# qitianwu/SGFormer

Hardware: NVIDIA H100
Metric: nodes/sec fwd+bwd (higher is better)
Workload: dtype bf16

## Files before the change

include/sgformer_b200.h:

```cpp
#ifndef SGFORMER_B200_H
#define SGFORMER_B200_H

#include <stddef.h>
#include <stdint.h>

#ifdef __cplusplus
extern "C" {
#endif

#define SGF_F32 0
#define SGF_BF16 1

#define SGF_ERR_ARG (-1)
#define SGF_ERR_UNSUPPORTED (-2)
#define SGF_ERR_DRIVER (-3)

const char* sgf_version(void);
int64_t sgf_launch_count(void);
int sgf_set_device(int device);

int sgf_csr_build_ws_bytes(int64_t nnz, int64_t n, size_t* bytes );
int sgf_csr_build(const int64_t* edge_index , int64_t nnz, int64_t n, int by_source,
                  int self_loop_mode, int64_t* rowptr , int32_t* col, float* dinv ,
                  void* ws, size_t ws_bytes, void* stream);
// ... 19 lines not shown
int sgf_add_self_loops(const int64_t* edge_index, int64_t nnz, int64_t n, int64_t* out_edge_index ,
                       void* stream);
int sgf_edge_symmetry(const int64_t* edge_index, int64_t nnz, int64_t n, uint64_t* out2, void* stream);
int sgf_csr_build_weighted_ws_bytes(int64_t nnz, int64_t n, size_t* bytes );
int sgf_csr_build_weighted(const int64_t* edge_index, const float* weight , int64_t nnz, int64_t n, int by_source,
                           int self_loop_mode, int64_t* rowptr, int32_t* col, int64_t* eid, float* val, float* dinv ,
                           void* ws, size_t ws_bytes, void* stream);
int sgf_edge_symmetry_weighted(const int64_t* edge_index, const float* weight, int64_t nnz, int64_t n, uint64_t* out2, void* stream);
int sgf_edge_weight_grad(const int64_t* rowptr, const int32_t* col, const int64_t* eid, int64_t n_rows, int h, int dtype,
                         const void* a, int64_t lda, const void* b, int64_t ldb, const void* y, int64_t ldy, const void* u, int64_t ldu,
                         const float* dinv, const int64_t* edge_index, int64_t nnz, float* loop_grad, float* out, void* stream);
int sgf_csr_subset_ws_bytes(int64_t n_sub, int64_t max_out_nnz, size_t* bytes);
int sgf_csr_subset(const int64_t* rowptr, const int32_t* col, int64_t n, const int64_t* subset, int64_t n_sub,
                   int32_t* node_map, int64_t* out_rowptr , int32_t* out_col, int64_t out_col_capacity,
                   float* dinv , int64_t* out_needed, void* ws, size_t ws_bytes, void* stream);

int sgf_spmm(const int64_t* rowptr, const int32_t* col, const float* row_scale, const void* x, int64_t ldx,
             void* y, int64_t ldy, int64_t n_rows, int h, int dtype,
             int64_t max_row_len ,
             void* stream);
int sgf_spmm_heavy(const int32_t* col, const float* row_scale, const void* x, int64_t ldx, void* y, int64_t ldy, int h,
                   int dtype, const int64_t* seg_start, const int32_t* seg_len, int64_t n_seg, float* partial,
                   const int64_t* heavy_rows, const int64_t* heavy_seg_ptr, int64_t n_heavy, void* stream);
int sgf_spmm_weighted(const int64_t* rowptr, const int32_t* col, const float* val, const float* row_scale, const void* x, int64_t ldx,
                      void* y, int64_t ldy, int64_t n_rows, int h, int dtype, int64_t max_row_len, void* stream);
int sgf_spmm_heavy_weighted(const int32_t* col, const float* val, const float* row_scale, const void* x, int64_t ldx, void* y,
                            int64_t ldy, int h, int dtype, const int64_t* seg_start, const int32_t* seg_len, int64_t n_seg,
                            float* partial, const int64_t* heavy_rows, const int64_t* heavy_seg_ptr, int64_t n_heavy, void* stream);
int sgf_spmm_sum(const int64_t* rowptr, const int32_t* col, const void* x, int64_t ldx, void* y, int64_t ldy, int64_t n_rows, int h,
                 int dtype, int64_t max_row_len, void* stream);
int sgf_spmm_heavy_sum(const int32_t* col, const void* x, int64_t ldx, void* y, int64_t ldy, int h, int dtype,
                       const int64_t* seg_start, const int32_t* seg_len, int64_t n_seg, float* partial, const int64_t* heavy_rows,
                       const int64_t* heavy_seg_ptr, int64_t n_heavy, void* stream);

#define SGF_GAT_MAX_HEADS 8
int sgf_gat_logits(const void* xp, int64_t ldx, int64_t n, int heads, int c, int dtype, const float* att_src, const float* att_dst,
                   float* a_src, float* a_dst, void* stream);
int sgf_gat_fwd(const int64_t* rowptr, const int32_t* col, const void* xp, int64_t ldx, const float* a_src, const float* a_dst,
                int64_t n, int heads, int c, int dtype, int mean, const float* bias, void* out, int64_t ldo, float* lse, float p,
                uint64_t seed, void* stream);
int sgf_gat_bwd(const int64_t* rowptr, const int32_t* col, const int64_t* rowptr_t, const int32_t* col_t, const void* xp, int64_t ldx,
                const float* a_src, const float* a_dst, const float* lse, const void* g, int64_t ldg, const float* att_src,
                const float* att_dst, int64_t n, int heads, int c, int dtype, int mean, float p, uint64_t seed, float* r_ws,
                float* da_src, float* da_dst, void* dxp, int64_t ldd, void* stream);
int sgf_dense_dropout(const float* x, int64_t ldx, int64_t rows, int64_t cols, float p, uint64_t seed, float* y, int64_t ldy,
                      void* stream);

int sgf_spmm_flagged(const int64_t* rowptr, const int32_t* col, const float* row_scale, const void* x, int64_t ldx, void* y,
                     int64_t ldy, int64_t n_rows, int h, int dtype, int64_t max_row_len, const uint32_t* flags, int64_t slot_rows,
                     int n_slots, void* stream);
int sgf_spmm_range(const int64_t* rowptr, const int32_t* col, const float* row_scale, const void* x, int64_t ldx, void* y,
                   int64_t ldy, int64_t n_rows, int h, int dtype, const int32_t* lo, const int32_t* hi, const float* part_in,
                   float* part_out, int64_t ld_part, void* stream);
int sgf_csr_row_splits(const int64_t* rowptr, const int32_t* col, int64_t n_rows, const int32_t* thresholds, int n_thr,
                       int32_t* splits, void* stream);
int sgf_signal(uint32_t* flag, uint32_t value, void* stream);
int sgf_memcpy_async(void* dst, const void* src, size_t bytes, void* stream);
int sgf_wait_flags(const uint32_t* flags, int n, void* stream);

#define SGF_MAX_SRC 4
#define SGF_MAX_SEG 16

#define SGF_EPI_AFFINE 0
#define SGF_EPI_ATTN_APPLY 1
#define SGF_EPI_ATTN_GRAM 2

// ... 176 lines not shown
```

sgformer_b200/_lib.py:

```python
import ctypes as C
import os

from . import _build

_i32, _i64, _f32, _u64, _vp, _sz = C.c_int32, C.c_int64, C.c_float, C.c_uint64, C.c_void_p, C.c_size_t
SGF_MAX_SRC, SGF_MAX_SEG = 4, 16
F32, BF16 = 0, 1
EPI_AFFINE, EPI_ATTN_APPLY, EPI_ATTN_GRAM = 0, 1, 2


class GemmNtArgs(C.Structure):
    _fields_ = [
        ("a", _vp * SGF_MAX_SRC), ("lda", _i64 * SGF_MAX_SRC), ("a_cols", _i64 * SGF_MAX_SRC),
        ("b", _vp * SGF_MAX_SRC), ("ldb", _i64 * SGF_MAX_SRC), ("b_cols", _i64 * SGF_MAX_SRC),
        ("n_a", _i32), ("n_b", _i32), ("n_seg", _i32),
        ("seg_a", _i32 * SGF_MAX_SEG), ("seg_akoff", _i32 * SGF_MAX_SEG), ("seg_b", _i32 * SGF_MAX_SEG),
        ("seg_bkoff", _i32 * SGF_MAX_SEG), ("seg_klen", _i32 * SGF_MAX_SEG),
        ("b_tail", _vp), ("ldb_tail", _i64),
        ("rows", _i64), ("n_out", _i32),
        ("epi", _i32),
        ("out", _vp), ("ldo", _i64), ("out_dtype", _i32),
        ("bias", _vp),
        ("aux", _vp), ("ld_aux", _i64), ("aux_dtype", _i32),
        ("row_scale", _vp),
# ... 109 lines not shown
    "sgf_bn_bwd_apply": (C.c_int, [_vp, _vp, _vp, _vp, _i64, _i64, C.c_int, C.c_int, _vp, _vp, _vp, _vp, _vp, C.c_int,
                                   C.c_int, C.c_int, _f32, _u64, _f32, _i64, _vp, _vp, _vp, C.c_int, _vp, _vp, _vp, _sz, _vp]),
    "sgf_bn_fwd_jk": (C.c_int, [_vp, _i64, _i64, C.c_int, C.c_int, _vp, _vp, _vp, _vp, _vp, C.c_int, C.c_int, _f32, _u64, _vp,
                                C.c_int, _vp, _i64, _vp, C.c_int, _vp]),
    "sgf_bn_bwd_reduce_jk": (C.c_int, [_vp, _vp, _i64, _i64, C.c_int, C.c_int, _vp, _vp, _vp, _vp, _vp, C.c_int, C.c_int, _f32,
                                       _u64, _vp, C.c_int, _vp, _i64, _vp, C.c_int, _vp, _sz, _vp]),
    "sgf_bn_bwd_apply_jk": (C.c_int, [_vp, _vp, _i64, _i64, C.c_int, C.c_int, _vp, _vp, _vp, _vp, _vp, C.c_int, C.c_int,
                                      C.c_int, _f32, _u64, _vp, _vp, _vp, _vp, C.c_int, _vp, _i64, _vp, C.c_int, _vp, _sz, _vp]),
    "sgf_axpby": (C.c_int, [_vp, _i64, C.c_int, _vp, _i64, C.c_int, _f32, _f32, _vp, _vp, _i64, C.c_int, _i64, C.c_int,
                            _vp]),
    "sgf_pack_operand": (C.c_int, [_vp, _i64, _i64, C.c_int, C.c_int, _vp, _i64, C.c_int, _i64, _vp, _vp, _vp, _sz, _vp]),
    "sgf_csr_subset_ws_bytes": (C.c_int, [_i64, _i64, C.POINTER(_sz)]),
    "sgf_csr_subset": (C.c_int, [_vp, _vp, _i64, _vp, _i64, _vp, _vp, _vp, _i64, _vp, _vp, _vp, _sz, _vp]),
    "sgf_eval_acc": (C.c_int, [_vp, _i64, _vp, _vp, _i64, _i64, C.c_int, _vp, _vp, _vp]),
    "sgf_softmax_nll": (C.c_int, [_vp, _i64, _vp, _vp, _i64, C.c_int, _f32, _vp, _vp, _i64, _vp, _sz, _vp]),
    "sgf_head_mean": (C.c_int, [_vp, _i64, _i64, C.c_int, C.c_int, C.c_int, _vp, _i64, _vp]),
    "sgf_attn_prepare_fwd": (C.c_int, [_vp, _vp, _vp, C.c_int, _vp, C.c_int, C.c_int, C.c_int, _vp, _i64, _vp, _i64,
                                       _i64, _vp, _vp]),
    "sgf_attn_bwd_prep": (C.c_int, [_vp, _i64, _vp, _i64, _vp, _i64, C.c_int, C.c_int, _f32, _vp, _i64, _vp, _vp]),
    "sgf_attn_combine_scal": (C.c_int, [_vp, C.c_int, C.c_int, _vp, _vp]),
    "sgf_gat_logits": (C.c_int, [_vp, _i64, _i64, C.c_int, C.c_int, C.c_int, _vp, _vp, _vp, _vp, _vp]),
    "sgf_gat_fwd": (C.c_int, [_vp, _vp, _vp, _i64, _vp, _vp, _i64, C.c_int, C.c_int, C.c_int, C.c_int, _vp, _vp, _i64, _vp, _f32,
                              _u64, _vp]),
    "sgf_gat_bwd": (C.c_int, [_vp, _vp, _vp, _vp, _vp, _i64, _vp, _vp, _vp, _vp, _i64, _vp, _vp, _i64, C.c_int, C.c_int, C.c_int,
                              C.c_int, _f32, _u64, _vp, _vp, _vp, _vp, _i64, _vp]),
    "sgf_dense_dropout": (C.c_int, [_vp, _i64, _i64, _i64, _f32, _u64, _vp, _i64, _vp]),
    "sgf_csr_build_weighted_ws_bytes": (C.c_int, [_i64, _i64, C.POINTER(_sz)]),
    "sgf_csr_build_weighted": (C.c_int, [_vp, _vp, _i64, _i64, C.c_int, C.c_int, _vp, _vp, _vp, _vp, _vp, _vp, _sz, _vp]),
    "sgf_edge_symmetry_weighted": (C.c_int, [_vp, _vp, _i64, _i64, _vp, _vp]),
    "sgf_spmm_weighted": (C.c_int, [_vp, _vp, _vp, _vp, _vp, _i64, _vp, _i64, _i64, C.c_int, C.c_int, _i64, _vp]),
    "sgf_spmm_heavy_weighted": (C.c_int, [_vp, _vp, _vp, _vp, _i64, _vp, _i64, C.c_int, C.c_int, _vp, _vp, _i64, _vp, _vp, _vp,
                                          _i64, _vp]),
    "sgf_spmm_sum": (C.c_int, [_vp, _vp, _vp, _i64, _vp, _i64, _i64, C.c_int, C.c_int, _i64, _vp]),
    "sgf_spmm_heavy_sum": (C.c_int, [_vp, _vp, _i64, _vp, _i64, C.c_int, C.c_int, _vp, _vp, _i64, _vp, _vp, _vp, _i64, _vp]),
    "sgf_edge_weight_grad": (C.c_int, [_vp, _vp, _vp, _i64, C.c_int, C.c_int, _vp, _i64, _vp, _i64, _vp, _i64, _vp, _i64, _vp,
                                       _vp, _i64, _vp, _vp, _vp]),
    "sgf_attn_prepare_bwd": (C.c_int, [_vp, _vp, _vp, _vp, _vp, C.c_int, C.c_int, _vp, _i64, _vp, _i64, _vp, _i64, _i64,
                                       _i64, _vp, _vp, _vp, _vp]),
}

_lib = None


def lib_path():
    return _build.LIB_PATH


def load():
    global _lib
    if _lib is None:
        path = lib_path()
        if not os.path.exists(path):
            raise RuntimeError(
                f"sgformer_b200: CUDA library not built ({path} missing). Run `python -c 'import __graft_entry__ as g; "
                "g.build()'` at the repo root. There is no CPU fallback.")
        lib = C.CDLL(path)
        for name, (res, args) in _SIGS.items():
            fn = getattr(lib, name)
            fn.restype, fn.argtypes = res, args
        _lib = lib
    return _lib


_CUDA_ERRORS = {1: "invalid value", 2: "out of memory", 98: "invalid device function", 209: "no kernel image for device",
                700: "illegal address", 701: "launch out of resources", 716: "misaligned address", 719: "launch failure",
                35: "driver too old", 100: "no CUDA device", 101: "invalid device"}
# ... 10 lines not shown
```

sgformer_b200/csrc/spmm.cu:

```cuda
#include "common.cuh"
#include "launch_count.h"
#include "../../include/sgformer_b200.h"

namespace sgf {

constexpr int kSpmmBlock = 256;
#ifndef SGF_SPMM_UNROLL
#define SGF_SPMM_UNROLL 4
#endif
#ifndef SGF_SPMM_MIN_BLOCKS
#define SGF_SPMM_MIN_BLOCKS 4
#endif
#ifndef SGF_SPMM_PIPELINE
#define SGF_SPMM_PIPELINE 0
#endif
constexpr int kUnroll = SGF_SPMM_UNROLL;
constexpr int kMinBlocks = SGF_SPMM_MIN_BLOCKS;

template <typename T, int CPL, bool COH = false, bool WEIGHTED = false>
__device__ __forceinline__ void gather_item(int my_idx, int cnt, const T* __restrict__ x, int64_t ldx, int groups, int grp,
                                            const int (&coff)[CPL], const bool (&cval)[CPL], float (&acc)[CPL][Vec16<T>::N],
                                            float my_w = 0.f) {
    constexpr int VN = Vec16<T>::N;
    for (int j0 = 0; j0 < cnt; j0 += groups * kUnroll) {
        uint4 v[kUnroll][CPL];
        int nb[kUnroll];
        float wt[kUnroll];
#pragma unroll
        for (int u = 0; u < kUnroll; ++u) {
            int j = j0 + u * groups + grp;
            int t = __shfl_sync(0xffffffffu, my_idx, j & 31);
            nb[u] = j < cnt ? t : -1;
            if constexpr (WEIGHTED) wt[u] = __shfl_sync(0xffffffffu, my_w, j & 31);
        }
#pragma unroll
        for (int u = 0; u < kUnroll; ++u) {
            const T* src = x + (int64_t)(nb[u] < 0 ? 0 : nb[u]) * ldx;
#pragma unroll
            for (int c = 0; c < CPL; ++c) {
                if (nb[u] >= 0 && cval[c]) v[u][c] = COH ? ldg_na(src + coff[c]) : ldg_nc_na(src + coff[c]);
                else v[u][c] = make_uint4(0u, 0u, 0u, 0u);
            }
        }
#pragma unroll
        for (int u = 0; u < kUnroll; ++u)
#pragma unroll
            for (int c = 0; c < CPL; ++c) {
                float f[VN];
                Vec16<T>::unpack(v[u][c], f);
                if constexpr (WEIGHTED) {
#pragma unroll
                    for (int i = 0; i < VN; ++i) acc[c][i] = fmaf(wt[u], f[i], acc[c][i]);
                } else {
#pragma unroll
                    for (int i = 0; i < VN; ++i) acc[c][i] += f[i];
                }
            }
    }
}

template <typename T, int CPL, bool WEIGHTED = false>
__device__ __forceinline__ void gather_range(const int32_t* __restrict__ col, const T* __restrict__ x, int64_t ldx, int64_t s, int64_t e,
                                             int lane, int groups, int grp, const int (&coff)[CPL], const bool (&cval)[CPL],
                                             float (&acc)[CPL][Vec16<T>::N], const float* __restrict__ val = nullptr) {
    for (int64_t base = s; base < e; base += 32) {
        const int cnt = (int)((e - base) < 32 ? (e - base) : 32);
        const int my_idx = lane < cnt ? ldg_nc_na_s32(col + base + lane) : -1;
        if constexpr (WEIGHTED) {
            const float my_w = lane < cnt ? __ldg(val + base + lane) : 0.f;
            gather_item<T, CPL, false, true>(my_idx, cnt, x, ldx, groups, grp, coff, cval, acc, my_w);
        } else {
            gather_item<T, CPL>(my_idx, cnt, x, ldx, groups, grp, coff, cval, acc);
        }
    }
}

struct SlotWait {
    const uint32_t* flags;
    int64_t slot_rows;
    int n_slots;
};
__device__ __forceinline__ int wait_slots(int need, volatile int* s_ready, int* s_lock, const uint32_t* flags) {
    uint32_t spins = 0;
    while (true) {
        const int r = *s_ready;
        if (r >= need) { __threadfence_block(); return r; }
        if (atomicCAS(s_lock, 0, 1) == 0) {
            int got = *s_ready;
            while (got < need && ld_acquire_sys_u32(flags + got + 1) != 0u) ++got;
            if (got > r) atomicMax(const_cast<int*>(s_ready), got);
            __threadfence_block();
            atomicExch(s_lock, 0);
            if (got >= need) return got;
            __nanosleep(400);
        } else {
            __nanosleep(200);
        }
        if (++spins > (1u << 24)) __trap();
    }
}
template <typename T, int CPL>
__device__ __forceinline__ void gather_range_flagged(const int32_t* __restrict__ col, const T* __restrict__ x, int64_t ldx, int64_t s,
                                                     int64_t e, int lane, int groups, int grp, const int (&coff)[CPL],
                                                     const bool (&cval)[CPL], float (&acc)[CPL][Vec16<T>::N], const SlotWait& sw,
                                                     int& ready, volatile int* s_ready, int* s_lock) {
// ... 53 lines not shown
#pragma unroll
            for (int c = 0; c < CPL; ++c)
#pragma unroll
                for (int i = 0; i < VN; ++i) acc[c][i] += __shfl_xor_sync(0xffffffffu, acc[c][i], o);
        }
        if (grp == 0) {
#pragma unroll
            for (int c = 0; c < CPL; ++c) {
                if (!cval[c]) continue;
                if (rr.part_in) {
                    const float4* pi = reinterpret_cast<const float4*>(rr.part_in + r * rr.ld_part + coff[c]);
#pragma unroll
                    for (int q = 0; q < VN / 4; ++q) {
                        const float4 v = pi[q];
                        acc[c][4 * q] += v.x; acc[c][4 * q + 1] += v.y; acc[c][4 * q + 2] += v.z; acc[c][4 * q + 3] += v.w;
                    }
                }
                if (rr.part_out) {
                    float4* po = reinterpret_cast<float4*>(rr.part_out + r * rr.ld_part + coff[c]);
#pragma unroll
                    for (int q = 0; q < VN / 4; ++q) po[q] = make_float4(acc[c][4 * q], acc[c][4 * q + 1], acc[c][4 * q + 2], acc[c][4 * q + 3]);
                } else {
                    const float rs = row_scale ? row_scale[r] : 1.0f;
                    float f[VN];
#pragma unroll
                    for (int i = 0; i < VN; ++i) f[i] = acc[c][i] * rs;
                    stg_na(y + r * ldy + coff[c], Vec16<T>::pack(f));
                }
            }
        }
    }
}

template <typename T, int CPL, bool FLAGS = false, bool WEIGHTED = false, bool SCALED = true>
__global__ void __launch_bounds__(kSpmmBlock, kMinBlocks)
spmm_rows_kernel(const int64_t* __restrict__ rowptr, const int32_t* __restrict__ col, const float* __restrict__ row_scale,
                 const T* __restrict__ x, int64_t ldx, T* __restrict__ y, int64_t ldy, int64_t n_rows, int chunks, int lpr_log2,
                 int64_t max_len, SlotWait sw, const float* __restrict__ val = nullptr) {
    constexpr int VN = Vec16<T>::N;
    __shared__ int s_ready, s_lock;
    int ready = 0;
    if (FLAGS) {
        if (threadIdx.x == 0) { s_ready = 0; s_lock = 0; }
        __syncthreads();
    }
    const int lane = threadIdx.x & 31;
    const int lpr = 1 << lpr_log2;
    const int groups = 32 >> lpr_log2;
    const int grp = lane >> lpr_log2;
    const int sub = lane & (lpr - 1);
    const int64_t warp0 = ((int64_t)blockIdx.x * kSpmmBlock + threadIdx.x) >> 5;
    const int64_t nwarps = ((int64_t)gridDim.x * kSpmmBlock) >> 5;
    int coff[CPL];
    bool cval[CPL];
#pragma unroll
    for (int c = 0; c < CPL; ++c) {
        int ch = sub + c * lpr;
        cval[c] = ch < chunks;
        coff[c] = ch * VN;
    }
#if SGF_SPMM_PIPELINE
    static_assert(!FLAGS && !WEIGHTED, "the flagged and weighted variants use the simple loop");
    int64_t r = warp0;
    if (r >= n_rows) return;
    int64_t s = rowptr[r], e = rowptr[r + 1];
    bool skip = max_len > 0 && e - s > max_len;
    if (skip) e = s;
    int64_t rn = r + nwarps, sn = 0, en = 0;
    if (rn < n_rows) { sn = rowptr[rn]; en = rowptr[rn + 1]; }
    int64_t base = s;
    int idx = (base + lane < e) ? ldg_nc_na_s32(col + base + lane) : -1;
// ... 31 lines not shown
                    T* dst = y + r * ldy;
#pragma unroll
                    for (int c = 0; c < CPL; ++c) {
                        if (!cval[c]) continue;
                        float f[VN];
#pragma unroll
                        for (int i = 0; i < VN; ++i) f[i] = SCALED ? acc[c][i] * rs : acc[c][i];
                        stg_na(dst + coff[c], Vec16<T>::pack(f));
                    }
                }
            }
            if (rn >= n_rows) break;
            r = rn; s = sn; e = ne; skip = nskip;
            rn = rnn; sn = snn; en = enn;
#pragma unroll
            for (int c = 0; c < CPL; ++c)
#pragma unroll
                for (int i = 0; i < VN; ++i) acc[c][i] = 0.f;
        }
        base = nbase;
        idx = nidx;
    }
#else
    for (int64_t r = warp0; r < n_rows; r += nwarps) {
        const int64_t s = rowptr[r];
        const int64_t e = rowptr[r + 1];
        if (max_len > 0 && e - s > max_len) continue;
        float acc[CPL][VN];
#pragma unroll
        for (int c = 0; c < CPL; ++c)
#pragma unroll
            for (int i = 0; i < VN; ++i) acc[c][i] = 0.f;
        if (FLAGS) gather_range_flagged<T, CPL>(col, x, ldx, s, e, lane, groups, grp, coff, cval, acc, sw, ready, &s_ready, &s_lock);
        else gather_range<T, CPL, WEIGHTED>(col, x, ldx, s, e, lane, groups, grp, coff, cval, acc, val);
        for (int o = lpr; o < 32; o <<= 1) {
#pragma unroll
            for (int c = 0; c < CPL; ++c)
#pragma unroll
                for (int i = 0; i < VN; ++i) acc[c][i] += __shfl_xor_sync(0xffffffffu, acc[c][i], o);
        }
        const float rs = (SCALED && row_scale) ? row_scale[r] : 1.0f;
        if (grp == 0) {
            T* dst = y + r * ldy;
#pragma unroll
            for (int c = 0; c < CPL; ++c) {
                if (!cval[c]) continue;
                float f[VN];
#pragma unroll
                for (int i = 0; i < VN; ++i) f[i] = SCALED ? acc[c][i] * rs : acc[c][i];
                stg_na(dst + coff[c], Vec16<T>::pack(f));
            }
        }
    }
#endif
}

template <typename T, int CPL, bool WEIGHTED = false>
__global__ void __launch_bounds__(kSpmmBlock, kMinBlocks)
spmm_segments_kernel(const int32_t* __restrict__ col, const T* __restrict__ x, int64_t ldx, const int64_t* __restrict__ seg_start,
                     const int32_t* __restrict__ seg_len, int64_t n_seg, float* __restrict__ partial, int h, int chunks,
                     int lpr_log2, const float* __restrict__ val = nullptr) {
    constexpr int VN = Vec16<T>::N;
    const int lane = threadIdx.x & 31;
    const int lpr = 1 << lpr_log2;
    const int groups = 32 >> lpr_log2;
    const int grp = lane >> lpr_log2;
    const int sub = lane & (lpr - 1);
// ... 38 lines not shown
                                           const float* __restrict__ row_scale, T* __restrict__ y, int64_t ldy, int h) {
    const int64_t total = n_heavy * h;
    for (int64_t t = (int64_t)blockIdx.x * blockDim.x + threadIdx.x; t < total; t += (int64_t)gridDim.x * blockDim.x) {
        const int64_t i = t / h;
        const int c = (int)(t - i * h);
        float s = 0.f;
        for (int64_t sg = heavy_seg_ptr[i]; sg < heavy_seg_ptr[i + 1]; ++sg) s += partial[sg * h + c];
        const int64_t r = heavy_rows[i];
        y[r * ldy + c] = from_f32<T>(SCALED ? s * (row_scale ? row_scale[r] : 1.f) : s);
    }
}

template <typename T, bool SCALED = true>
static int launch_spmm(const int64_t* rowptr, const int32_t* col, const float* row_scale, const void* x, int64_t ldx,
                       void* y, int64_t ldy, int64_t n_rows, int h, int64_t max_len, cudaStream_t st, const SlotWait* slots = nullptr,
                       const float* val = nullptr) {
    constexpr int VN = Vec16<T>::N;
    if (h % VN != 0 || ldx % VN != 0 || ldy % VN != 0) return SGF_ERR_ARG;
    if ((reinterpret_cast<uintptr_t>(x) & 15) || (reinterpret_cast<uintptr_t>(y) & 15)) return SGF_ERR_ARG;
    const int chunks = h / VN;
    int lpr_log2 = 0;
    while ((1 << lpr_log2) < chunks && lpr_log2 < 5) ++lpr_log2;
    const int lpr = 1 << lpr_log2;
    const int cpl = (chunks + lpr - 1) / lpr;
    if (n_rows == 0) return SGF_OK;
    int64_t warps_needed = n_rows;
    int64_t blocks = (warps_needed * 32 + kSpmmBlock - 1) / kSpmmBlock;
    int64_t cap = (int64_t)num_sms() * kMinBlocks * 8;
    if (blocks > cap) blocks = cap;
    if (slots && blocks > (int64_t)num_sms() * kMinBlocks) blocks = (int64_t)num_sms() * kMinBlocks;
    const T* xp = static_cast<const T*>(x);
    T* yp = static_cast<T*>(y);
    const SlotWait sw = slots ? *slots : SlotWait{nullptr, 1, 1};
#define SGF_SPMM_CASE(N)                                                                                              \
    case N:                                                                                                           \
        if (slots)                                                                                                    \
            spmm_rows_kernel<T, N, true><<<(unsigned)blocks, kSpmmBlock, 0, st>>>(rowptr, col, row_scale, xp, ldx, yp, ldy, \
                                                                                  n_rows, chunks, lpr_log2, max_len, sw);   \
        else if (val)                                                                                                 \
            spmm_rows_kernel<T, N, false, true><<<(unsigned)blocks, kSpmmBlock, 0, st>>>(rowptr, col, row_scale, xp, ldx, yp, \
                                                                                   ldy, n_rows, chunks, lpr_log2, max_len, sw, val); \
        else                                                                                                          \
            spmm_rows_kernel<T, N, false, false, SCALED><<<(unsigned)blocks, kSpmmBlock, 0, st>>>(                   \
                rowptr, col, row_scale, xp, ldx, yp, ldy, n_rows, chunks, lpr_log2, max_len, sw);                        \
        break;
    switch (cpl) {
        SGF_SPMM_CASE(1)
        SGF_SPMM_CASE(2)
        SGF_SPMM_CASE(3)
        SGF_SPMM_CASE(4)
        default: return SGF_ERR_UNSUPPORTED;
    }
#undef SGF_SPMM_CASE
    SGF_LAUNCH_CHECK();
    count_launch();
    return SGF_OK;
}

template <typename T>
static int launch_range(const int64_t* rowptr, const int32_t* col, const float* row_scale, const void* x, int64_t ldx, void* y,
                        int64_t ldy, int64_t n_rows, int h, const RowRange& rr, cudaStream_t st) {
    constexpr int VN = Vec16<T>::N;
    if (h % VN != 0 || ldx % VN != 0 || (y && ldy % VN != 0) || rr.ld_part % 4 != 0) return SGF_ERR_ARG;
    if ((reinterpret_cast<uintptr_t>(x) & 15) || (reinterpret_cast<uintptr_t>(y) & 15) || (reinterpret_cast<uintptr_t>(rr.part_in) & 15) ||
        (reinterpret_cast<uintptr_t>(rr.part_out) & 15))
        return SGF_ERR_ARG;
    const int chunks = h / VN;
    int lpr_log2 = 0;
    while ((1 << lpr_log2) < chunks && lpr_log2 < 5) ++lpr_log2;
    const int lpr = 1 << lpr_log2;
    const int cpl = (chunks + lpr - 1) / lpr;
    if (n_rows == 0) return SGF_OK;
    int64_t blocks = (n_rows * 32 + kSpmmBlock - 1) / kSpmmBlock;
    int64_t cap = (int64_t)num_sms() * kMinBlocks * 8;
    if (blocks > cap) blocks = cap;
    const T* xp = static_cast<const T*>(x);
    T* yp = static_cast<T*>(y);
// ... 29 lines not shown
    const int cpl = (chunks + lpr - 1) / lpr;
    int64_t blocks = (n_seg * 32 + kSpmmBlock - 1) / kSpmmBlock;
    int64_t cap = (int64_t)num_sms() * kMinBlocks * 8;
    if (blocks > cap) blocks = cap;
    const T* xp = static_cast<const T*>(x);
#define SGF_SEG_CASE(N)                                                                                                 \
    case N:                                                                                                             \
        if (val)                                                                                                        \
            spmm_segments_kernel<T, N, true><<<(unsigned)blocks, kSpmmBlock, 0, st>>>(col, xp, ldx, seg_start, seg_len, n_seg, \
                                                                                      partial, h, chunks, lpr_log2, val); \
        else                                                                                                            \
            spmm_segments_kernel<T, N><<<(unsigned)blocks, kSpmmBlock, 0, st>>>(col, xp, ldx, seg_start, seg_len, n_seg, \
                                                                                partial, h, chunks, lpr_log2);          \
        break;
    switch (cpl) {
        SGF_SEG_CASE(1)
        SGF_SEG_CASE(2)
        SGF_SEG_CASE(3)
        SGF_SEG_CASE(4)
        default: return SGF_ERR_UNSUPPORTED;
    }
#undef SGF_SEG_CASE
    SGF_LAUNCH_CHECK();
    count_launch();
    int64_t fb = (n_heavy * h + 255) / 256;
    if (fb > cap) fb = cap;
    spmm_heavy_finalize_kernel<T, SCALED><<<(unsigned)fb, 256, 0, st>>>(partial, heavy_rows, heavy_seg_ptr, n_heavy, row_scale,
                                                                static_cast<T*>(y), ldy, h);
    SGF_LAUNCH_CHECK();
    count_launch();
    return SGF_OK;
}

__global__ void signal_kernel(uint32_t* flag, uint32_t value) { st_release_sys_u32(flag, value); }
__global__ void wait_flags_kernel(const uint32_t* flags, int n) {
    uint32_t spins = 0;
    for (int i = threadIdx.x; i < n; i += blockDim.x)
        while (ld_acquire_sys_u32(flags + i) == 0u) {
            __nanosleep(500);
            if (++spins > (1u << 24)) __trap();
        }
}

}

extern "C" int sgf_spmm_flagged(const int64_t* rowptr, const int32_t* col, const float* row_scale, const void* x, int64_t ldx,
                                void* y, int64_t ldy, int64_t n_rows, int h, int dtype, int64_t max_row_len, const uint32_t* flags,
                                int64_t slot_rows, int n_slots, void* stream) {
    if (!rowptr || n_rows < 0 || h <= 0 || (n_rows > 0 && (!x || !y)) || max_row_len < 0 || !flags || slot_rows <= 0 || n_slots < 1)
        return SGF_ERR_ARG;
    cudaStream_t st = (cudaStream_t)stream;
    const sgf::SlotWait sw{flags, slot_rows, n_slots};
    if (dtype == 0) return sgf::launch_spmm<float>(rowptr, col, row_scale, x, ldx, y, ldy, n_rows, h, max_row_len, st, &sw);
    if (dtype == 1) return sgf::launch_spmm<__nv_bfloat16>(rowptr, col, row_scale, x, ldx, y, ldy, n_rows, h, max_row_len, st, &sw);
    return SGF_ERR_ARG;
}

extern "C" int sgf_spmm_range(const int64_t* rowptr, const int32_t* col, const float* row_scale, const void* x, int64_t ldx, void* y,
                              int64_t ldy, int64_t n_rows, int h, int dtype, const int32_t* lo, const int32_t* hi,
                              const float* part_in, float* part_out, int64_t ld_part, void* stream) {
    if (!rowptr || n_rows < 0 || h <= 0 || (n_rows > 0 && !x) || (!part_out && n_rows > 0 && !y)) return SGF_ERR_ARG;
    if ((part_in || part_out) && ld_part < h) return SGF_ERR_ARG;
    const sgf::RowRange rr{lo, hi, part_in, part_out, ld_part};
    cudaStream_t st = (cudaStream_t)stream;
    if (dtype == 0) return sgf::launch_range<float>(rowptr, col, row_scale, x, ldx, y, ldy, n_rows, h, rr, st);
    if (dtype == 1) return sgf::launch_range<__nv_bfloat16>(rowptr, col, row_scale, x, ldx, y, ldy, n_rows, h, rr, st);
// ... 70 lines not shown
    if (dtype == 0)
        return sgf::launch_heavy<float>(col, row_scale, x, ldx, y, ldy, h, seg_start, seg_len, n_seg, partial, heavy_rows,
                                        heavy_seg_ptr, n_heavy, st, val);
    if (dtype == 1)
        return sgf::launch_heavy<__nv_bfloat16>(col, row_scale, x, ldx, y, ldy, h, seg_start, seg_len, n_seg, partial, heavy_rows,
                                                heavy_seg_ptr, n_heavy, st, val);
    return SGF_ERR_ARG;
}

extern "C" int sgf_spmm_sum(const int64_t* rowptr, const int32_t* col, const void* x, int64_t ldx, void* y, int64_t ldy,
                            int64_t n_rows, int h, int dtype, int64_t max_row_len, void* stream) {
    if (!rowptr || n_rows < 0 || h <= 0 || (n_rows > 0 && (!col || !x || !y)) || max_row_len < 0) return SGF_ERR_ARG;
    cudaStream_t st = (cudaStream_t)stream;
    if (dtype == 0) return sgf::launch_spmm<float, false>(rowptr, col, nullptr, x, ldx, y, ldy, n_rows, h, max_row_len, st);
    if (dtype == 1) return sgf::launch_spmm<__nv_bfloat16, false>(rowptr, col, nullptr, x, ldx, y, ldy, n_rows, h, max_row_len, st);
    return SGF_ERR_ARG;
}

extern "C" int sgf_spmm_heavy_sum(const int32_t* col, const void* x, int64_t ldx, void* y, int64_t ldy, int h, int dtype,
                                  const int64_t* seg_start, const int32_t* seg_len, int64_t n_seg, float* partial,
                                  const int64_t* heavy_rows, const int64_t* heavy_seg_ptr, int64_t n_heavy, void* stream) {
    if (!col || !x || !y || h <= 0 || n_seg < 0 || n_heavy < 0) return SGF_ERR_ARG;
    if (n_seg == 0 || n_heavy == 0) return SGF_OK;
    if (!seg_start || !seg_len || !partial || !heavy_rows || !heavy_seg_ptr) return SGF_ERR_ARG;
    cudaStream_t st = (cudaStream_t)stream;
    if (dtype == 0)
        return sgf::launch_heavy<float, false>(col, nullptr, x, ldx, y, ldy, h, seg_start, seg_len, n_seg, partial, heavy_rows,
                                               heavy_seg_ptr, n_heavy, st);
    if (dtype == 1)
        return sgf::launch_heavy<__nv_bfloat16, false>(col, nullptr, x, ldx, y, ldy, h, seg_start, seg_len, n_seg, partial,
                                                       heavy_rows, heavy_seg_ptr, n_heavy, st);
    return SGF_ERR_ARG;
}
```

sgformer_b200/kernels.py:

```python
from __future__ import annotations

import ctypes as C
import os
import threading
from dataclasses import dataclass
from typing import Optional, Sequence, Tuple

import torch

from . import _lib
from ._lib import BF16, EPI_AFFINE, EPI_ATTN_APPLY, EPI_ATTN_GRAM, F32, AttnGramArgs, GemmNtArgs, GemmTnArgs, check

Tensor = torch.Tensor
_tls = threading.local()


def lib():
    return _lib.load()


def _use(t: Tensor):
    if not t.is_cuda:
        raise RuntimeError("sgformer_b200 kernels need CUDA tensors (no CPU fallback); got device " + str(t.device))
    idx = t.device.index if t.device.index is not None else torch.cuda.current_device()
# ... 294 lines not shown
                                   _p(heavy.seg_len), ns, _p(partial), _p(heavy.rows), _p(heavy.seg_ptr), heavy.rows.numel(),
                                   _stream()), "sgf_spmm_heavy")
    if ev is not None:
        e1.record()
        ev.append((e0, e1))
    return out


def spmm_sum(rowptr: Tensor, col: Tensor, x: Tensor, out: Optional[Tensor] = None, heavy: Optional[HeavyRows] = None) -> Tensor:
    _use(x)
    n = rowptr.numel() - 1
    rows, h, ldx = _mat(x, "x")
    if out is None:
        out = alloc_act(n, h, x.dtype, x.device)
    _, ho, ldy = _mat(out, "out")
    if ho != h or out.dtype != x.dtype:
        raise ValueError("spmm_sum: out shape/dtype mismatch")
    ev = spmm_events
    if ev is not None:
        e0, e1 = torch.cuda.Event(enable_timing=True), torch.cuda.Event(enable_timing=True)
        e0.record()
    check(lib().sgf_spmm_sum(_p(rowptr), _p(col), _p(x), ldx, _p(out), ldy, n, h, dcode(x), HEAVY_ROW if heavy is not None else 0,
                             _stream()), "sgf_spmm_sum")
    if heavy is not None:
        ns = heavy.seg_start.numel()
        partial = torch.empty((ns, h), dtype=torch.float32, device=x.device)
        check(lib().sgf_spmm_heavy_sum(_p(col), _p(x), ldx, _p(out), ldy, h, dcode(x), _p(heavy.seg_start), _p(heavy.seg_len), ns,
                                       _p(partial), _p(heavy.rows), _p(heavy.seg_ptr), heavy.rows.numel(), _stream()),
              "sgf_spmm_heavy_sum")
    if ev is not None:
        e1.record()
        ev.append((e0, e1))
    return out


def _spmm_weighted(rowptr: Tensor, col: Tensor, val: Tensor, row_scale: Optional[Tensor], x: Tensor, out: Optional[Tensor],
                   heavy: Optional[HeavyRows]) -> Tensor:
    _use(x)
    n = rowptr.numel() - 1
    rows, h, ldx = _mat(x, "x")
    if val.dtype != torch.float32 or not val.is_contiguous() or val.numel() != col.numel():
        raise ValueError("spmm: val must be contiguous fp32 with one value per column id")
    if out is None:
        out = alloc_act(n, h, x.dtype, x.device)
    _, ho, ldy = _mat(out, "out")
    if ho != h or out.dtype != x.dtype:
        raise ValueError("spmm: out shape/dtype mismatch")
    ev = spmm_events
    if ev is not None:
        e0, e1 = torch.cuda.Event(enable_timing=True), torch.cuda.Event(enable_timing=True)
        e0.record()
    rs = _f32vec(row_scale, n, "row_scale")
    check(lib().sgf_spmm_weighted(_p(rowptr), _p(col), _p(val), _p(rs), _p(x), ldx, _p(out), ldy, n, h, dcode(x),
                                  HEAVY_ROW if heavy is not None else 0, _stream()), "sgf_spmm_weighted")
    if heavy is not None:
        ns = heavy.seg_start.numel()
        partial = torch.empty((ns, h), dtype=torch.float32, device=x.device)
        check(lib().sgf_spmm_heavy_weighted(_p(col), _p(val), _p(rs), _p(x), ldx, _p(out), ldy, h, dcode(x), _p(heavy.seg_start),
                                            _p(heavy.seg_len), ns, _p(partial), _p(heavy.rows), _p(heavy.seg_ptr),
                                            heavy.rows.numel(), _stream()), "sgf_spmm_heavy_weighted")
    if ev is not None:
        e1.record()
        ev.append((e0, e1))
    return out


# ... 817 lines not shown
```

Before: 12.66 million.

## Add L2 evict-last hints for hot rows and a column-blocked tiled SpMM

In the default row SpMM (single-chunk-per-lane case), gathers from the first rows of x, sized to fit a fixed L2 budget, now use an L2 evict_last policy and all other rows use evict_first. This only applies when the feature matrix exceeds a size threshold, and is meant to keep a stable hot subset resident in L2 during random neighbour gathers. Separately, it adds a tiled SpMM that converts x to a slice-major layout, splits edges into source-column blocks and accumulates partial sums in shared memory across blocks. It also adds a plan builder and a random-gather probe kernel. The tiled path adds a layout-conversion pass and plan memory, and nothing in the shown code calls it by default.

Result: faster. 12.83 million (median of 6 runs) (+1.4%).

```diff
diff --git a/include/sgformer_b200.h b/include/sgformer_b200.h
--- a/include/sgformer_b200.h
+++ b/include/sgformer_b200.h
@@ -75,6 +75,11 @@
 int sgf_spmm_heavy_sum(const int32_t* col, const void* x, int64_t ldx, void* y, int64_t ldy, int h, int dtype,
                        const int64_t* seg_start, const int32_t* seg_len, int64_t n_seg, float* partial, const int64_t* heavy_rows,
                        const int64_t* heavy_seg_ptr, int64_t n_heavy, void* stream);
+
+int sgf_spmm_tiled(const int32_t* boff, const int32_t* bcol, int n_blocks, int64_t n_src, const float* row_scale, int scaled,
+                   const void* x, int64_t ldx, void* xs, void* y, int64_t ldy, int64_t n_rows, int h, int dtype, int tile,
+                   int max_ctas, void* stream);
+int sgf_gather_probe(const void* buf, int64_t footprint, int iters, int64_t threads, uint32_t* sink, void* stream);
 
 #define SGF_GAT_MAX_HEADS 8
 int sgf_gat_logits(const void* xp, int64_t ldx, int64_t n, int heads, int c, int dtype, const float* att_src, const float* att_dst,
diff --git a/sgformer_b200/_lib.py b/sgformer_b200/_lib.py
--- a/sgformer_b200/_lib.py
+++ b/sgformer_b200/_lib.py
@@ -165,6 +165,9 @@
     "sgf_spmm_heavy_weighted": (C.c_int, [_vp, _vp, _vp, _vp, _i64, _vp, _i64, C.c_int, C.c_int, _vp, _vp, _i64, _vp, _vp, _vp,
                                           _i64, _vp]),
     "sgf_spmm_sum": (C.c_int, [_vp, _vp, _vp, _i64, _vp, _i64, _i64, C.c_int, C.c_int, _i64, _vp]),
+    "sgf_spmm_tiled": (C.c_int, [_vp, _vp, C.c_int, _i64, _vp, C.c_int, _vp, _i64, _vp, _vp, _i64, _i64, C.c_int, C.c_int, C.c_int,
+                                 C.c_int, _vp]),
+    "sgf_gather_probe": (C.c_int, [_vp, _i64, C.c_int, _i64, _vp, _vp]),
     "sgf_spmm_heavy_sum": (C.c_int, [_vp, _vp, _i64, _vp, _i64, C.c_int, C.c_int, _vp, _vp, _i64, _vp, _vp, _vp, _i64, _vp]),
     "sgf_edge_weight_grad": (C.c_int, [_vp, _vp, _vp, _i64, C.c_int, C.c_int, _vp, _i64, _vp, _i64, _vp, _i64, _vp, _i64, _vp,
                                        _vp, _i64, _vp, _vp, _vp]),
diff --git a/sgformer_b200/csrc/spmm.cu b/sgformer_b200/csrc/spmm.cu
--- a/sgformer_b200/csrc/spmm.cu
+++ b/sgformer_b200/csrc/spmm.cu
@@ -17,11 +17,46 @@
 constexpr int kUnroll = SGF_SPMM_UNROLL;
 constexpr int kMinBlocks = SGF_SPMM_MIN_BLOCKS;
 
-template <typename T, int CPL, bool COH = false, bool WEIGHTED = false>
+__device__ __forceinline__ uint64_t policy_evict_last() {
+    uint64_t p;
+    asm volatile("createpolicy.fractional.L2::evict_last.b64 %0, 1.0;" : "=l"(p));
+    return p;
+}
+__device__ __forceinline__ uint64_t policy_evict_first() {
+    uint64_t p;
+    asm volatile("createpolicy.fractional.L2::evict_first.b64 %0, 1.0;" : "=l"(p));
+    return p;
+}
+__device__ __forceinline__ uint4 ldg_nc_na_hint(const void* p, uint64_t pol) {
+    uint4 r;
+    asm volatile("ld.global.nc.L1::no_allocate.L2::cache_hint.v4.u32 {%0,%1,%2,%3}, [%4], %5;"
+                 : "=r"(r.x), "=r"(r.y), "=r"(r.z), "=r"(r.w) : "l"(p), "l"(pol));
+    return r;
+}
+__device__ __forceinline__ int ldg_nc_s32_hint(const int* p, uint64_t pol) {
+    int r;
+    asm volatile("ld.global.nc.L2::cache_hint.s32 %0, [%1], %2;" : "=r"(r) : "l"(p), "l"(pol));
+    return r;
+}
+__device__ __forceinline__ void stg_na_hint(void* p, const uint4& v, uint64_t pol) {
+    asm volatile("st.global.L1::no_allocate.L2::cache_hint.v4.u32 [%0], {%1,%2,%3,%4}, %5;"
+                 :: "l"(p), "r"(v.x), "r"(v.y), "r"(v.z), "r"(v.w), "l"(pol) : "memory");
+}
+
+#ifndef SGF_SPMM_HOT_MB
+#define SGF_SPMM_HOT_MB 24
+#endif
+constexpr int64_t kHotMinBytes = (int64_t)512 << 20;
+template <typename T, int CPL, bool COH = false, bool WEIGHTED = false, bool HOT = false>
 __device__ __forceinline__ void gather_item(int my_idx, int cnt, const T* __restrict__ x, int64_t ldx, int groups, int grp,
                                             const int (&coff)[CPL], const bool (&cval)[CPL], float (&acc)[CPL][Vec16<T>::N],
-                                            float my_w = 0.f) {
-    constexpr int VN = Vec16<T>::N;
+                                            float my_w = 0.f, int hot_rows = -1) {
+    constexpr int VN = Vec16<T>::N;
+    uint64_t pol_hot = 0, pol_cold = 0;
+    if constexpr (HOT) {
+        pol_hot = policy_evict_last();
+        pol_cold = policy_evict_first();
+    }
     for (int j0 = 0; j0 < cnt; j0 += groups * kUnroll) {
         uint4 v[kUnroll][CPL];
         int nb[kUnroll];
@@ -38,8 +73,13 @@
             const T* src = x + (int64_t)(nb[u] < 0 ? 0 : nb[u]) * ldx;
 #pragma unroll
             for (int c = 0; c < CPL; ++c) {
-                if (nb[u] >= 0 && cval[c]) v[u][c] = COH ? ldg_na(src + coff[c]) : ldg_nc_na(src + coff[c]);
-                else v[u][c] = make_uint4(0u, 0u, 0u, 0u);
+                if (nb[u] >= 0 && cval[c]) {
+                    if constexpr (COH) v[u][c] = ldg_na(src + coff[c]);
+                    else if constexpr (HOT) v[u][c] = ldg_nc_na_hint(src + coff[c], nb[u] < hot_rows ? pol_hot : pol_cold);
+                    else v[u][c] = ldg_nc_na(src + coff[c]);
+                } else {
+                    v[u][c] = make_uint4(0u, 0u, 0u, 0u);
+                }
             }
         }
 #pragma unroll
@@ -59,10 +99,11 @@
     }
 }
 
-template <typename T, int CPL, bool WEIGHTED = false>
+template <typename T, int CPL, bool WEIGHTED = false, bool HOT = false>
 __device__ __forceinline__ void gather_range(const int32_t* __restrict__ col, const T* __restrict__ x, int64_t ldx, int64_t s, int64_t e,
                                              int lane, int groups, int grp, const int (&coff)[CPL], const bool (&cval)[CPL],
-                                             float (&acc)[CPL][Vec16<T>::N], const float* __restrict__ val = nullptr) {
+                                             float (&acc)[CPL][Vec16<T>::N], const float* __restrict__ val = nullptr,
+                                             int hot_rows = -1) {
     for (int64_t base = s; base < e; base += 32) {
         const int cnt = (int)((e - base) < 32 ? (e - base) : 32);
         const int my_idx = lane < cnt ? ldg_nc_na_s32(col + base + lane) : -1;
@@ -70,7 +111,7 @@
             const float my_w = lane < cnt ? __ldg(val + base + lane) : 0.f;
             gather_item<T, CPL, false, true>(my_idx, cnt, x, ldx, groups, grp, coff, cval, acc, my_w);
         } else {
-            gather_item<T, CPL>(my_idx, cnt, x, ldx, groups, grp, coff, cval, acc);
+            gather_item<T, CPL, false, false, HOT>(my_idx, cnt, x, ldx, groups, grp, coff, cval, acc, 0.f, hot_rows);
         }
     }
 }
@@ -190,11 +231,11 @@
     }
 }
 
-template <typename T, int CPL, bool FLAGS = false, bool WEIGHTED = false, bool SCALED = true>
+template <typename T, int CPL, bool FLAGS = false, bool WEIGHTED = false, bool SCALED = true, bool HOT = false>
 __global__ void __launch_bounds__(kSpmmBlock, kMinBlocks)
 spmm_rows_kernel(const int64_t* __restrict__ rowptr, const int32_t* __restrict__ col, const float* __restrict__ row_scale,
                  const T* __restrict__ x, int64_t ldx, T* __restrict__ y, int64_t ldy, int64_t n_rows, int chunks, int lpr_log2,
-                 int64_t max_len, SlotWait sw, const float* __restrict__ val = nullptr) {
+                 int64_t max_len, SlotWait sw, int hot_rows, const float* __restrict__ val = nullptr) {
     constexpr int VN = Vec16<T>::N;
     __shared__ int s_ready, s_lock;
     int ready = 0;
@@ -292,7 +333,7 @@
 #pragma unroll
             for (int i = 0; i < VN; ++i) acc[c][i] = 0.f;
         if (FLAGS) gather_range_flagged<T, CPL>(col, x, ldx, s, e, lane, groups, grp, coff, cval, acc, sw, ready, &s_ready, &s_lock);
-        else gather_range<T, CPL, WEIGHTED>(col, x, ldx, s, e, lane, groups, grp, coff, cval, acc, val);
+        else gather_range<T, CPL, WEIGHTED, HOT>(col, x, ldx, s, e, lane, groups, grp, coff, cval, acc, val, hot_rows);
         for (int o = lpr; o < 32; o <<= 1) {
 #pragma unroll
             for (int c = 0; c < CPL; ++c)
@@ -397,17 +438,26 @@
     const T* xp = static_cast<const T*>(x);
     T* yp = static_cast<T*>(y);
     const SlotWait sw = slots ? *slots : SlotWait{nullptr, 1, 1};
+    const int64_t row_bytes = (int64_t)h * (int64_t)sizeof(T);
+    int hot_rows = -1;
+    if (SGF_SPMM_HOT_MB > 0 && n_rows * row_bytes >= kHotMinBytes) {
+        const int64_t hr = ((int64_t)SGF_SPMM_HOT_MB << 20) / (ldx * (int64_t)sizeof(T));
+        hot_rows = (int)(hr < n_rows ? hr : n_rows);
+    }
 #define SGF_SPMM_CASE(N)                                                                                              \
     case N:                                                                                                           \
         if (slots)                                                                                                    \
             spmm_rows_kernel<T, N, true><<<(unsigned)blocks, kSpmmBlock, 0, st>>>(rowptr, col, row_scale, xp, ldx, yp, ldy, \
-                                                                                  n_rows, chunks, lpr_log2, max_len, sw);   \
+                                                                                  n_rows, chunks, lpr_log2, max_len, sw, -1); \
         else if (val)                                                                                                 \
             spmm_rows_kernel<T, N, false, true><<<(unsigned)blocks, kSpmmBlock, 0, st>>>(rowptr, col, row_scale, xp, ldx, yp, \
-                                                                                   ldy, n_rows, chunks, lpr_log2, max_len, sw, val); \
+                                                                                   ldy, n_rows, chunks, lpr_log2, max_len, sw, -1, val); \
+        else if (N == 1 && hot_rows >= 0)                                                                             \
+            spmm_rows_kernel<T, N, false, false, SCALED, true><<<(unsigned)blocks, kSpmmBlock, 0, st>>>(             \
+                rowptr, col, row_scale, xp, ldx, yp, ldy, n_rows, chunks, lpr_log2, max_len, sw, hot_rows);              \
         else                                                                                                          \
             spmm_rows_kernel<T, N, false, false, SCALED><<<(unsigned)blocks, kSpmmBlock, 0, st>>>(                   \
-                rowptr, col, row_scale, xp, ldx, yp, ldy, n_rows, chunks, lpr_log2, max_len, sw);                        \
+                rowptr, col, row_scale, xp, ldx, yp, ldy, n_rows, chunks, lpr_log2, max_len, sw, -1);                    \
         break;
     switch (cpl) {
         SGF_SPMM_CASE(1)
@@ -503,6 +553,161 @@
     return SGF_OK;
 }
 
+constexpr int kTiledBlock = 512;
+constexpr int kTiledUnroll = 4;
+#ifndef SGF_TILED_HINTS
+#define SGF_TILED_HINTS 1
+#endif
+
+template <typename T>
+__global__ void slice_major_kernel(const T* __restrict__ x, int64_t ldx, T* __restrict__ xs, int64_t n, int chunks) {
+    constexpr int VN = Vec16<T>::N;
+    const uint64_t pol = policy_evict_first();
+    const int64_t total = n * chunks;
+    for (int64_t q = (int64_t)blockIdx.x * blockDim.x + threadIdx.x; q < total; q += (int64_t)gridDim.x * blockDim.x) {
+        const int64_t r = q / chunks;
+        const int c = (int)(q - r * chunks);
+        const uint4 v = ldg_nc_na(x + r * ldx + (int64_t)c * VN);
+        stg_na_hint(xs + ((int64_t)(c >> 1) * n + r) * (2 * VN) + (c & 1) * VN, v, pol);
+    }
+}
+
+template <typename T, bool SCALED>
+__global__ void __launch_bounds__(kTiledBlock, 2)
+spmm_tiled_kernel(const int32_t* __restrict__ boff, const int32_t* __restrict__ bcol, int n_blocks, const float* __restrict__ row_scale,
+                  const T* __restrict__ xs, int64_t n_src, T* __restrict__ y, int64_t ldy, int64_t n_rows, int n_slices, int tile) {
+    constexpr int VN = Vec16<T>::N;
+    extern __shared__ float4 s_acc4[];
+    float* s_acc = reinterpret_cast<float*>(s_acc4);
+    const int lane = threadIdx.x & 31;
+    const int warp = threadIdx.x >> 5;
+    const int half = lane & 1;
+    constexpr int kWarps = kTiledBlock / 32;
+    const uint64_t pol_keep = policy_evict_last();
+    const uint64_t pol_stream = policy_evict_first();
+    const int64_t n_tiles = (n_rows + tile - 1) / tile;
+    const int64_t n_units = n_tiles * n_slices;
+    for (int64_t u = blockIdx.x; u < n_units; u += gridDim.x) {
+        const int sl = (int)(u / n_tiles);
+        const int64_t r0 = (u - (int64_t)sl * n_tiles) * tile;
+        const int rows = (int)((n_rows - r0) < tile ? (n_rows - r0) : tile);
+        const T* xsl = xs + (int64_t)sl * n_src * (2 * VN) + half * VN;
+        for (int b = 0; b < n_blocks; ++b) {
+            const int32_t* off = boff + (int64_t)b * n_rows + r0;
+            for (int i0 = warp * 16; i0 < rows; i0 += kWarps * 16) {
+                const int i = i0 + (lane >> 1);
+                const bool ok = i < rows;
+                int s = 0, len = 0;
+                if (ok) { s = ldg_nc_s32_hint(off + i, pol_stream); len = ldg_nc_s32_hint(off + i + 1, pol_stream) - s; }
+                float acc[VN];
+                float* sa = s_acc + (int64_t)i * (2 * VN) + half * VN;
+                if (b == 0 || !ok) {
+#pragma unroll
+                    for (int k = 0; k < VN; ++k) acc[k] = 0.f;
+                } else {
+#pragma unroll
+                    for (int k = 0; k < VN; k += 4) {
+                        const float4 v = *reinterpret_cast<const float4*>(sa + k);
+                        acc[k] = v.x; acc[k + 1] = v.y; acc[k + 2] = v.z; acc[k + 3] = v.w;
+                    }
+                }
+                const int maxlen = __reduce_max_sync(0xffffffffu, len);
+                for (int j0 = 0; j0 < maxlen; j0 += kTiledUnroll) {
+                    int nb[kTiledUnroll];
+#pragma unroll
+                    for (int k = 0; k < kTiledUnroll; ++k)
+                        nb[k] = j0 + k >= len ? -1 : SGF_TILED_HINTS ? ldg_nc_s32_hint(bcol + s + j0 + k, pol_stream) : __ldg(bcol + s + j0 + k);
+                    uint4 v[kTiledUnroll];
+#pragma unroll
+                    for (int k = 0; k < kTiledUnroll; ++k)
+                        v[k] = nb[k] < 0 ? make_uint4(0u, 0u, 0u, 0u)
+                               : SGF_TILED_HINTS ? ldg_nc_na_hint(xsl + (int64_t)nb[k] * (2 * VN), pol_keep) : ldg_nc_na(xsl + (int64_t)nb[k] * (2 * VN));
+#pragma unroll
+                    for (int k = 0; k < kTiledUnroll; ++k) {
+                        if (nb[k] < 0) continue;
+                        float f[VN];
+                        Vec16<T>::unpack(v[k], f);
+#pragma unroll
+                        for (int q = 0; q < VN; ++q) acc[q] += f[q];
+                    }
+                }
+                if (!ok) continue;
+                if (b + 1 < n_blocks) {
+#pragma unroll
+                    for (int k = 0; k < VN; k += 4) *reinterpret_cast<float4*>(sa + k) = make_float4(acc[k], acc[k + 1], acc[k + 2], acc[k + 3]);
+                } else {
+                    const int64_t r = r0 + i;
+                    const float rs = (SCALED && row_scale) ? row_scale[r] : 1.0f;
+                    float f[VN];
+#pragma unroll
+                    for (int q = 0; q < VN; ++q) f[q] = SCALED ? acc[q] * rs : acc[q];
+                    stg_na_hint(y + r * ldy + (int64_t)sl * (2 * VN) + half * VN, Vec16<T>::pack(f), pol_stream);
+                }
+            }
+        }
+    }
+}
+
+static int tiled_default_tile(int slice_floats) {
+    int dev = 0, smem = 0;
+    if (cudaGetDevice(&dev) != cudaSuccess || cudaDeviceGetAttribute(&smem, cudaDevAttrMaxSharedMemoryPerMultiprocessor, dev) != cudaSuccess)
+        smem = 228 * 1024;
+    const int per_cta = smem / 2 - 2048;
+    return (per_cta / (slice_floats * 4)) / 16 * 16;
+}
+
+template <typename T, bool SCALED>
+static int launch_tiled(const int32_t* boff, const int32_t* bcol, int n_blocks, int64_t n_src, const float* row_scale, const void* x,
+                        int64_t ldx, void* xs, void* y, int64_t ldy, int64_t n_rows, int h, int tile, int max_ctas, cudaStream_t st) {
+    constexpr int VN = Vec16<T>::N;
+    if (h % (2 * VN) != 0 || ldx % VN != 0 || ldy % VN != 0 || ldx < h || ldy < h) return SGF_ERR_ARG;
+    if ((reinterpret_cast<uintptr_t>(x) & 15) || (reinterpret_cast<uintptr_t>(y) & 15) || (reinterpret_cast<uintptr_t>(xs) & 31))
+        return SGF_ERR_ARG;
+    if (n_rows == 0) return SGF_OK;
+    const int chunks = h / VN;
+    const int n_slices = chunks / 2;
+    const int slice_floats = 2 * VN;
+    if (tile <= 0) tile = tiled_default_tile(slice_floats);
+    if (tile % 16 != 0) return SGF_ERR_ARG;
+    const size_t smem = (size_t)tile * slice_floats * sizeof(float);
+    auto kern = spmm_tiled_kernel<T, SCALED>;
+    SGF_CUDA_TRY(cudaFuncSetAttribute(kern, cudaFuncAttributeMaxDynamicSharedMemorySize, (int)smem));
+    int64_t tb = (n_src * chunks + 255) / 256;
+    const int64_t tcap = (int64_t)num_sms() * 16;
+    slice_major_kernel<T><<<(unsigned)(tb < tcap ? tb : tcap), 256, 0, st>>>(static_cast<const T*>(x), ldx, static_cast<T*>(xs), n_src,
+                                                                             chunks);
+    SGF_LAUNCH_CHECK();
+    count_launch();
+    const int64_t units = ((n_rows + tile - 1) / tile) * n_slices;
+    int64_t grid = (int64_t)num_sms() * 2;
+    if (max_ctas > 0 && grid > max_ctas) grid = max_ctas;
+    if (grid > units) grid = units;
+    kern<<<(unsigned)grid, kTiledBlock, smem, st>>>(boff, bcol, n_blocks, row_scale, static_cast<const T*>(xs), n_src, static_cast<T*>(y),
+                                                    ldy, n_rows, n_slices, tile);
+    SGF_LAUNCH_CHECK();
+    count_launch();
+    return SGF_OK;
+}
+
+__global__ void gather_probe_kernel(const uint4* __restrict__ buf, int64_t n_sectors, int iters, uint32_t* __restrict__ sink) {
+    const uint64_t pol = policy_evict_last();
+    const int half = threadIdx.x & 1;
+    uint32_t h = (uint32_t)(blockIdx.x * blockDim.x + threadIdx.x) >> 1;
+    uint32_t x = 0;
+    for (int it = 0; it < iters; it += 4) {
+        uint4 v[4];
+#pragma unroll
+        for (int k = 0; k < 4; ++k) {
+            h = h * 1664525u + 1013904223u;
+            const int64_t sec = (int64_t)(((uint64_t)(h ^ (h >> 15)) * (uint64_t)n_sectors) >> 32);
+            v[k] = ldg_nc_na_hint(buf + sec * 2 + half, pol);
+        }
+#pragma unroll
+        for (int k = 0; k < 4; ++k) x ^= v[k].x ^ v[k].y ^ v[k].z ^ v[k].w;
+    }
+    if (x == 0x9e3779b9u) sink[0] = x;
+}
+
 __global__ void signal_kernel(uint32_t* flag, uint32_t value) { st_release_sys_u32(flag, value); }
 __global__ void wait_flags_kernel(const uint32_t* flags, int n) {
     uint32_t spins = 0;
@@ -639,3 +844,28 @@
                                                        heavy_rows, heavy_seg_ptr, n_heavy, st);
     return SGF_ERR_ARG;
 }
+
+extern "C" int sgf_spmm_tiled(const int32_t* boff, const int32_t* bcol, int n_blocks, int64_t n_src, const float* row_scale, int scaled,
+                              const void* x, int64_t ldx, void* xs, void* y, int64_t ldy, int64_t n_rows, int h, int dtype, int tile,
+                              int max_ctas, void* stream) {
+    if (!boff || n_blocks < 1 || n_rows < 0 || n_src < 0 || h <= 0 || (n_rows > 0 && (!x || !xs || !y || !bcol)) || tile < 0 || max_ctas < 0)
+        return SGF_ERR_ARG;
+    cudaStream_t st = (cudaStream_t)stream;
+    if (dtype == 0)
+        return scaled ? sgf::launch_tiled<float, true>(boff, bcol, n_blocks, n_src, row_scale, x, ldx, xs, y, ldy, n_rows, h, tile, max_ctas, st)
+                      : sgf::launch_tiled<float, false>(boff, bcol, n_blocks, n_src, nullptr, x, ldx, xs, y, ldy, n_rows, h, tile, max_ctas, st);
+    if (dtype == 1)
+        return scaled ? sgf::launch_tiled<__nv_bfloat16, true>(boff, bcol, n_blocks, n_src, row_scale, x, ldx, xs, y, ldy, n_rows, h, tile,
+                                                               max_ctas, st)
+                      : sgf::launch_tiled<__nv_bfloat16, false>(boff, bcol, n_blocks, n_src, nullptr, x, ldx, xs, y, ldy, n_rows, h, tile,
+                                                                max_ctas, st);
+    return SGF_ERR_ARG;
+}
+
+extern "C" int sgf_gather_probe(const void* buf, int64_t footprint, int iters, int64_t threads, uint32_t* sink, void* stream) {
+    if (!buf || !sink || footprint < 32 || iters <= 0 || iters % 4 != 0 || threads <= 0 || threads % 256 != 0) return SGF_ERR_ARG;
+    sgf::gather_probe_kernel<<<(unsigned)(threads / 256), 256, 0, (cudaStream_t)stream>>>(static_cast<const uint4*>(buf), footprint / 32,
+                                                                                          iters, sink);
+    SGF_LAUNCH_CHECK(); sgf::count_launch();
+    return SGF_OK;
+}
diff --git a/sgformer_b200/kernels.py b/sgformer_b200/kernels.py
--- a/sgformer_b200/kernels.py
+++ b/sgformer_b200/kernels.py
@@ -350,6 +350,68 @@
         e1.record()
         ev.append((e0, e1))
     return out
+
+
+@dataclass
+class TiledPlan:
+    boff: Tensor
+    bcol: Tensor
+    n_blocks: int
+    block_rows: int
+    n_src: int
+    tile: int = 0
+    max_ctas: int = 0
+
+
+def tiled_plan(rowptr: Tensor, col: Tensor, n_src: int, block_rows: int, tile: int = 0, max_ctas: int = 0) -> TiledPlan:
+    n = rowptr.numel() - 1
+    nnz = col.numel()
+    if nnz >= 2 ** 31:
+        raise ValueError("tiled_plan: int32 block offsets need nnz < 2^31")
+    n_blocks = max(1, (n_src + block_rows - 1) // block_rows)
+    lens = rowptr[1:] - rowptr[:-1]
+    row_of = torch.repeat_interleave(torch.arange(n, device=col.device), lens)
+    keep = (lens <= HEAVY_ROW)[row_of]
+    row_of = row_of[keep]
+    c = col[keep]
+    key = (c.to(torch.int64) // block_rows) * n + row_of
+    del row_of
+    boff = torch.zeros(n_blocks * n + 1, dtype=torch.int64, device=col.device)
+    boff[1:] = torch.cumsum(torch.bincount(key, minlength=n_blocks * n), 0)
+    order = torch.sort(key // n, stable=True).indices
+    del key
+    return TiledPlan(boff.to(torch.int32), c[order].contiguous(), n_blocks, block_rows, n_src, tile, max_ctas)
+
+
+def spmm_tiled(plan: TiledPlan, col: Tensor, row_scale: Optional[Tensor], x: Tensor, out: Optional[Tensor] = None,
+               scaled: bool = True, heavy: Optional[HeavyRows] = None) -> Tensor:
+    _use(x)
+    n = (plan.boff.numel() - 1) // plan.n_blocks
+    rows, h, ldx = _mat(x, "x")
+    if rows != plan.n_src or h * x.element_size() < 512:
+        raise ValueError("spmm_tiled: x must have plan.n_src rows of at least 512 bytes")
+    if out is None:
+        out = alloc_act(n, h, x.dtype, x.device)
+    _, ho, ldy = _mat(out, "out")
+    if ho != h or out.dtype != x.dtype:
+        raise ValueError("spmm_tiled: out shape/dtype mismatch")
+    rs = _f32vec(row_scale, n, "row_scale") if scaled else None
+    xs = torch.empty(rows * h, dtype=x.dtype, device=x.device)
+    check(lib().sgf_spmm_tiled(_p(plan.boff), _p(plan.bcol), plan.n_blocks, plan.n_src, _p(rs), int(scaled), _p(x), ldx, _p(xs),
+                               _p(out), ldy, n, h, dcode(x), plan.tile, plan.max_ctas, _stream()), "sgf_spmm_tiled")
+    if heavy is not None:
+        ns = heavy.seg_start.numel()
+        partial = torch.empty((ns, h), dtype=torch.float32, device=x.device)
+        fn = lib().sgf_spmm_heavy if scaled else lib().sgf_spmm_heavy_sum
+        args = ([_p(col), _p(rs)] if scaled else [_p(col)]) + [_p(x), ldx, _p(out), ldy, h, dcode(x), _p(heavy.seg_start),
+                                                               _p(heavy.seg_len), ns, _p(partial), _p(heavy.rows),
+                                                               _p(heavy.seg_ptr), heavy.rows.numel(), _stream()]
+        check(fn(*args), "sgf_spmm_heavy" if scaled else "sgf_spmm_heavy_sum")
+    return out
+
+
+def gather_probe(buf: Tensor, footprint: int, iters: int, threads: int, sink: Tensor) -> None:
+    check(lib().sgf_gather_probe(_p(buf), footprint, iters, threads, _p(sink), _stream()), "sgf_gather_probe")
 
 
 def _spmm_weighted(rowptr: Tensor, col: Tensor, val: Tensor, row_scale: Optional[Tensor], x: Tensor, out: Optional[Tensor],
```
